# DavidSevic/gpu-nbody-simulation

Hardware: AMD Instinct MI355X
Metric: body-steps/sec (higher is better)
Workload: dtype f32

## Files before the change

gpu-nbody-simulation_amd/csrc/bh_engine.hip:

```cpp
#include "../../include/bhgpu.h"

#include <hip/hip_runtime.h>

#include <algorithm>
#include <chrono>
#include <cmath>
#include <cstdio>
#include <cstdlib>
#include <cstring>
#include <string>
#include <type_traits>
#include <vector>

#include "bh_tree.hpp"
#include "bh_walk_exact.hpp"
#include "bh_walk_f64.hpp"
#include "bh_diag.hpp"
#include "bh_direct.hpp"
#include "bh_field.hpp"
#include "bh_init.hpp"
#include "bh_let.hpp"
#include "bh_migrate.hpp"
#include "bh_split.hpp"
#include "bh_moments.hpp"
#include "bh_radial.hpp"
#include "bh_neighbours.hpp"
#include "bh_pairs.hpp"
#include "bh_groups.hpp"
#include "bh_mst.hpp"
#include "bh_binaries.hpp"
#include "bh_walk_fast.h"
#include "bh_run_state.hpp"
#include "bh_queries_state.hpp"

using namespace bh;

#ifdef BHGPU_EXPERIMENTS
#include "../../scripts/experiments/bh_engine_hooks.hpp"
#else
struct ExpHooks {
    hipError_t create(int64_t) { return hipSuccess; }
    void walk_args(WalkFastArgs &) const {}
    void destroy(int64_t) {}
};
#endif

static thread_local std::string g_create_error;

struct bh_ctx : RunState {
    bh_config cfg{};
    int Dm = 0;
    enum class Mode { Exact, F64, Mixed, F32 };
    Mode mode = Mode::Exact;
    bool tree64() const { return mode == Mode::Exact || mode == Mode::F64; }
    bool state64() const { return mode != Mode::F32; }
    bool compat = true;
    double eps = 0.0, eps2 = 0.0;
    float eps2f = 0.f;
    bool exact_thresholds = false;
    int device = 0;
    hipStream_t stream = nullptr;
    bool own_stream = false;
    int64_t n = 0;
    int64_t internal_cap = 0, node_cap = 0;
    int64_t bfs_max = 12288;
    int exact_bpw = 0;
    int walk_split = 0;
    bool walk_asm = true;
    int sort_bucket = 1;
    uint64_t *splitters = nullptr;
    uint16_t *sort_dig = nullptr;
    int sort_direct = 1;
    int64_t sort_direct_max = kSortDirectMax;
    uint64_t *keys_scatter = nullptr;
    uint64_t *direct_list = nullptr, *direct_range_keys = nullptr;
    uint32_t *direct_count = nullptr;
    uint32_t direct_cap = 0, direct_subcap = 0;
    int direct_nsub = 1;
    int direct_slot = 0;
    struct SortRecord {
        bool valid = false, offered = false;
        int64_t n = 0;
        int nb = 0, nsub = 0;
        uint32_t len = 0, cap = 0, subcap = 0;
        const uint32_t *count = nullptr;
    } sort_rec;
    int build_items = 0;
    bool hilbert = false;
    bool chain_collapse = true;
    double *bslots = nullptr;

    void *pos = nullptr, *vel = nullptr, *mass = nullptr, *force = nullptr;
    void *pos2 = nullptr, *vel2 = nullptr, *mass2 = nullptr, *force2 = nullptr;
    uint32_t *orig = nullptr, *orig2 = nullptr;
    int reorder_every = 16;
    float2 *spos = nullptr;
    float4 *sstate = nullptr;
    float *smass = nullptr;
    uint64_t *keys[2] = {nullptr, nullptr};
    uint32_t *vals[2] = {nullptr, nullptr};
    uint64_t *keys_sorted = nullptr;
    uint32_t *perm = nullptr;
    uint32_t *radix_counts = nullptr, *bsum_sort = nullptr, *bsum_u32 = nullptr, *cnt = nullptr;
    uint64_t *coarse = nullptr;
    uint32_t *cell_first = nullptr;
    d3 *terms = nullptr, *bsum_d3 = nullptr;
    double *partial = nullptr, *box = nullptr;
    NodeD *gd = nullptr;
    LinkD *ld = nullptr;
    QuadF *qf = nullptr;
    NodeAux *aux = nullptr;
    int32_t *self_node = nullptr, *cell_depth = nullptr;
    uint32_t *com_pending = nullptr;
    TreeCounters *ctr = nullptr;

    int rank = 0, world = 1;
    bool let_mode = false, external_box = false;
    int64_t let_cap = 0, quads_local = 0;
    int64_t forest_base = 0;
    uint64_t *needmask = nullptr;
    uint32_t *let_tsum = nullptr, *let_outidx = nullptr;
    QuadF *let_send = nullptr;
    double *lbounds = nullptr, *all_bounds = nullptr;
    float2 *acc_part = nullptr;
    LetCounters *let_ctr = nullptr;
    int64_t *gid = nullptr;
    uint32_t *group_cost = nullptr;
    const void **walk_consts = nullptr;
    uint32_t *body_counts = nullptr;
    double *phi = nullptr;
    uint32_t *phi_counts = nullptr;
    double *diag_part = nullptr, *diag_out = nullptr;
    TsRecord *ts_part = nullptr, *ts_out = nullptr;
    MapState map;
    RadState rad;
    FieldState field;
    NbState nb;
    PairState pair;
    FofState fof;
    MstState mst;
    BinState bin;
    double *slots_save = nullptr;
    TreeCounters *ctr_save = nullptr;
    uint32_t *perm_save = nullptr;
    uint32_t *slot_of = nullptr;
    int64_t *direct_targets = nullptr;
    double2 *direct_out = nullptr;
    void *check_force = nullptr;
    uint32_t *check_counts = nullptr, *check_cost = nullptr;
    bool sort_pack = true;
    unsigned long long *orb_hist = nullptr;
    double *mig_send = nullptr, *mig_recv = nullptr;
    ExpHooks exp;

    std::vector<hipEvent_t> ev;
    hipEvent_t ev_step[2] = {nullptr, nullptr}, ev_build[2] = {nullptr, nullptr};
    hipEvent_t ev_grp[3] = {nullptr, nullptr, nullptr};
    hipEvent_t ev_let[3] = {nullptr, nullptr, nullptr};
    bool let_timed = false;
    int64_t steps_done = 0;
    int32_t last_nsteps = 0;
    int timed_pairs = 0;
    bool step_timed = false;

    std::vector<void *> allocs;
    uint64_t device_bytes = 0;
    std::string err;
};

using Mode = bh_ctx::Mode;
// ... 12 lines not shown
        if (e_ != hipSuccess)                                                                   \
            return fail((c), BH_ERR_DEVICE,                                                     \
                        std::string(#call) + ": " + hipGetErrorString(e_));                     \
    } while (0)

template <typename T>
int dev_alloc(bh_ctx *c, T **out, size_t count)
{
    void *p = nullptr;
    const size_t bytes = std::max<size_t>(count, 1) * sizeof(T);
    hipError_t e = hipMalloc(&p, bytes);
    if (e != hipSuccess)
        return fail(c, BH_ERR_DEVICE, std::string("hipMalloc(") + std::to_string(bytes) + "): " + hipGetErrorString(e));
    c->allocs.push_back(p);
    c->device_bytes += bytes;
    *out = static_cast<T *>(p);
    return BH_OK;
}

inline void dev_free(bh_ctx *c, void *p)
{
    if (!p) return;
    auto it = std::find(c->allocs.begin(), c->allocs.end(), p);
    if (it != c->allocs.end()) { c->allocs.erase(it); (void)hipFree(p); }
}

inline unsigned blocks_for(int64_t n, int per_block) { return (unsigned)((n + per_block - 1) / per_block); }

template <typename F>
void dispatch(F &&f) { f(); }
template <typename F, typename... B>
void dispatch(F &&f, bool b, B... rest)
{
    if (b) dispatch([&](auto... t) { f(std::true_type{}, t...); }, rest...);
    else dispatch([&](auto... t) { f(std::false_type{}, t...); }, rest...);
}

template <typename F>
void with_state(const bh_ctx *c, F &&f)
{
    if (c->state64()) f(double2{}); else f(float2{});
}

inline size_t force_bytes(const bh_ctx *c, int64_t n)
{
    return (size_t)std::max<int64_t>(n, 1) * 2 * (c->tree64() ? sizeof(double) : sizeof(float));
}

inline int64_t cell_span(const bh_ctx *c)
{
    return std::max<int64_t>(1, std::min<int64_t>(c->internal_cap, std::max<int64_t>(c->n - 1, 0) * (int64_t)std::max(1, c->Dm)));
}

void owned_range(const bh_ctx *c, int64_t *lo, int64_t *hi)
{
    if (c->let_mode) { *lo = 0; *hi = c->n; return; }
    const int64_t per = (c->n + c->world - 1) / c->world;
    const int64_t chunk = (per + kBlock - 1) / kBlock * kBlock;
    *lo = std::min<int64_t>(c->n, chunk * c->rank);
    *hi = std::min<int64_t>(c->n, chunk * (c->rank + 1));
}

constexpr int64_t kComClimbMaxBodies = 32768;
constexpr int64_t kSmallBuildBodies = 327680;
constexpr int64_t kMediumBuildBodies = 786432;
constexpr int kSmallItems = 2;

template <typename Real2, typename Real>
__global__ __launch_bounds__(kBlock) void reorder_state_kernel(uint32_t *__restrict__ perm, const Real2 *__restrict__ pos,
                                                                const Real2 *__restrict__ vel, const Real *__restrict__ mass,
                                                                const float2 *__restrict__ acc, const uint32_t *__restrict__ orig,
                                                                Real2 *__restrict__ pos2, Real2 *__restrict__ vel2,
                                                                Real *__restrict__ mass2, float2 *__restrict__ acc2,
                                                                uint32_t *__restrict__ orig2, int64_t n)
{
    const int64_t s = (int64_t)blockIdx.x * kBlock + threadIdx.x;
    if (s >= n) return;
    const uint32_t b = perm[s];
    pos2[s] = pos[b]; vel2[s] = vel[b]; mass2[s] = mass[b]; acc2[s] = acc[b];
    orig2[s] = orig ? orig[b] : b;
    perm[s] = (uint32_t)s;
}

static void launch_nodes_fast(bh_ctx *c, bool full_aux, hipStream_t st)
{
    dispatch([&](auto compat, auto full, auto chains) {
        constexpr bool kCollapse = decltype(chains)::value && !decltype(full)::value;
        hipLaunchKernelGGL((nodes_fast_kernel<decltype(compat)::value, decltype(full)::value, kCollapse>),
                           dim3(blocks_for(cell_span(c), kBlock)),
                           dim3(kBlock), 0, st, c->keys_sorted, c->coarse, c->cnt, c->cell_first, c->spos, c->smass, c->box,
                           c->terms, c->n, c->Dm, c->cfg.theta, c->internal_cap, c->qf, c->aux, c->ctr);
    }, c->compat, full_aux, c->chain_collapse && !(c->let_mode && c->world > 1));
}

void clean_slots(bh_ctx *c) { if (c->carry.slots_dirty) hipLaunchKernelGGL(bounds_slots_reset, dim3(1), dim3(kWave), 0, c->stream, c->bslots); }

template <int SI>
int enqueue_lsd_passes(hipStream_t st, uint64_t *const keys[2], uint32_t *const vals[2], uint32_t *counts, uint32_t *rows, int64_t n,
                       int bits, bool packed)
{
    constexpr int SB = kSortBits;
    const unsigned nbl = blocks_for(n, kBlock * SI);
    const int passes = (bits + SB - 1) / SB;
    int cur = 0;
    for (int p = 0; p < passes; ++p) {
        const int shift = p * SB;
        auto scatter = [&](auto kern) {
            hipLaunchKernelGGL(kern, dim3(nbl), dim3(kBlock), 0, st, keys[cur], packed ? nullptr : vals[cur], keys[cur ^ 1],
                               vals[cur ^ 1], counts, rows, n, shift, (int)nbl, nullptr, nullptr, nullptr, 0u, 0u, 1);
        };
        hipLaunchKernelGGL((radix_hist<SI, SB>), dim3(nbl), dim3(kBlock), 0, st, keys[cur], counts, n, shift, (int)nbl);
        hipLaunchKernelGGL(radix_rowscan, dim3(1 << SB), dim3(kBlock), 0, st, counts, rows, (int)nbl);
        if (!packed) scatter(radix_scatter_w<SI, SB>);
        else if (p + 1 == passes) scatter(radix_scatter_w<SI, SB, 2>);
        else scatter(radix_scatter_w<SI, SB, 1>);
        cur ^= 1;
    }
    return cur;
}

template <bool TREE64, bool STATE64 = TREE64, int ITEMS = kItems>
int enqueue_build_t(bh_ctx *c, bool may_reorder, bool time_groups)
{
    constexpr int TILE = kBlock * ITEMS;
    static_assert(!TREE64 || STATE64, "an fp64 tree is built from fp64 state");
    using Real2 = typename std::conditional<STATE64, double2, float2>::type;
    using Real = typename std::conditional<STATE64, double, float>::type;
    const int64_t n = c->n;
    const int Dm = c->Dm;
    hipStream_t st = c->stream;
    const Real2 *pos = static_cast<const Real2 *>(c->pos);
    const Real *mass = static_cast<const Real *>(c->mass);

    const bool from_walk = c->carry.slots_valid;
    double *slots = c->external_box ? nullptr : c->bslots;
    if (slots) {
        if (!from_walk) {
            const unsigned nbb = std::max(1u, std::min(1024u, blocks_for(n, kBlock)));
            clean_slots(c);
            hipLaunchKernelGGL((bounds_partial<Real2>), dim3(nbb), dim3(kBlock), 0, st, pos, n, slots);
        }
    }
    BuildDone done{n, slots != nullptr, false, false, false, false};

    if (n > 0) {
        const bool pack = Dm >= 1 && 2 * Dm <= kPackShift && n <= ((int64_t)1 << (64 - kPackShift))
                          && c->sort_pack;
        const bool single = pack && n >= 2 && n <= 4 * kBsThreads && c->sort_bucket == 1;
        const bool bucket = !single && pack && n >= 2 && n <= kBucketMaxNBig && (c->sort_bucket == 2 || (c->sort_bucket == 1 && c->carry.samples_n == n));
        const int nb = (n <= kBucketMaxN) ? kBuckets : kBucketsBig;
        const int ns = (nb == kBuckets) ? ((n > (int64_t)1 << 18) ? 2 * kBuckets : kBuckets)
                                        : ((n > (int64_t)3 << 20) ? kMaxSplitSamples : kBucketsBig);
        static_assert(kBucketMaxN == (int64_t)1 << 20 && kBucketMaxNBig == (int64_t)1 << 22, "BASELINE configs 3 and 4 fit");
        done.sort_bucket = bucket || single; done.sort_packed = pack;
        const bool direct = bucket && !TREE64 && c->sort_direct != 0 && c->carry.samples_n == n;
        SortDirect sd;
        BucketDirect bd;
        if (direct) {
            const uint32_t len = (uint32_t)((n + nb - 1) / nb);
            sd.count = c->direct_count + c->direct_slot * kDirectCounterWords;
            sd.count_next = c->direct_count + (c->direct_slot ^ 1) * kDirectCounterWords;
            sd.list = c->direct_list; sd.range_keys = c->direct_range_keys; sd.cap = c->direct_cap; sd.subcap = c->direct_subcap;
            sd.len = len; sd.nsub = c->direct_nsub;
            bd.count = sd.count; bd.list = sd.list; bd.range_keys = sd.range_keys; bd.keys = c->keys[0]; bd.scratch = c->keys_scatter;
            bd.n = n; bd.cap = sd.cap; bd.subcap = sd.subcap; bd.len = len; bd.nb = nb; bd.nsub = sd.nsub;
            c->direct_slot ^= 1;
        }
        {
            const unsigned nkb = blocks_for(n, kBlock);
            auto keys_launch = [&](auto fs, auto pk, auto hil) {
                constexpr bool H = decltype(hil)::value, P = decltype(pk)::value, F = decltype(fs)::value;
                const bool smp = P && bucket;
// ... 401 lines not shown
    kQuietCounters = 1,
    kQuietOutputs = 2,
    kQuietCostPerm = 4,
};

void swap_walk_outputs(bh_ctx *c) { std::swap(c->force, c->check_force); std::swap(c->body_counts, c->check_counts); std::swap(c->group_cost, c->check_cost); }
template <typename Body>
int quietly(bh_ctx *c, unsigned opts, Body body)
{
    constexpr size_t off = offsetof(TreeCounters, visits), ctr_bytes = sizeof(TreeCounters) - off, slot_doubles = (size_t)4 * kBoundSlots;
    if ((opts & kQuietCounters) && !c->ctr_save) { if (int rc = dev_alloc(c, &c->ctr_save, 1)) return rc; }
    if (!c->slots_save) { if (int rc = dev_alloc(c, &c->slots_save, slot_doubles)) return rc; }
    RunState saved = *c;
    if ((opts & kQuietCostPerm) && c->last.group_cost_valid && c->is.tree_valid && !c->last.cost_perm && c->n > 0) {
        if (!c->perm_save) { if (int rc = dev_alloc(c, &c->perm_save, (size_t)std::max<int64_t>(c->cfg.capacity, 1))) return rc; }
        BH_HIP(c, hipMemcpyAsync(c->perm_save, c->perm, (size_t)c->n * sizeof(uint32_t), hipMemcpyDeviceToDevice, c->stream));
        saved.costs_indexed_through(c->perm_save);
    }
    if (opts & kQuietCounters) BH_HIP(c, hipMemcpyAsync((char *)c->ctr_save + off, (char *)c->ctr + off, ctr_bytes, hipMemcpyDeviceToDevice, c->stream));
    BH_HIP(c, hipMemcpyAsync(c->slots_save, c->bslots, slot_doubles * sizeof(double), hipMemcpyDeviceToDevice, c->stream));
    if (opts & kQuietOutputs) swap_walk_outputs(c);
    const int rc = body();
    if (opts & kQuietOutputs) swap_walk_outputs(c);
    c->quiet_end(saved);
    BH_HIP(c, hipMemcpyAsync(c->bslots, c->slots_save, slot_doubles * sizeof(double), hipMemcpyDeviceToDevice, c->stream));
    if (opts & kQuietCounters) BH_HIP(c, hipMemcpyAsync((char *)c->ctr + off, (char *)c->ctr_save + off, ctr_bytes, hipMemcpyDeviceToDevice, c->stream));
    return rc;
}

}

#include "bh_queries_host.hpp"


extern "C" {

int bh_abi_version(void) { return BHGPU_ABI_VERSION; }

#ifndef BHGPU_BUILD_INFO
#define BHGPU_BUILD_INFO "digest=unknown flags=unknown"
#endif
const char *bh_build_info(void) { return BHGPU_BUILD_INFO; }

const char *bh_last_error(const bh_ctx *ctx) { return ctx ? ctx->err.c_str() : g_create_error.c_str(); }

int bh_create(const bh_config *cfg, bh_ctx **out)
{
    if (!cfg || !out) return fail(nullptr, BH_ERR_ARG, "bh_create: null argument");
    *out = nullptr;
    if (cfg->capacity < 0 || cfg->capacity > 0x7fffffffLL - 8)
        return fail(nullptr, BH_ERR_ARG, "bh_create: capacity out of range");
    if (cfg->max_depth < 1 || cfg->max_depth > 32)
        return fail(nullptr, BH_ERR_ARG, "bh_create: max_depth must be 1..32");
    if (!(cfg->theta > 0.0)) return fail(nullptr, BH_ERR_ARG, "bh_create: theta must be > 0");
    if (cfg->precision != BH_PRECISION_F64_EXACT && cfg->precision != BH_PRECISION_F32 &&
        cfg->precision != BH_PRECISION_MIXED && cfg->precision != BH_PRECISION_F64)
        return fail(nullptr, BH_ERR_ARG, "bh_create: unknown precision");
    int ndev = 0;
    if (hipGetDeviceCount(&ndev) != hipSuccess || ndev <= 0)
        return fail(nullptr, BH_ERR_NO_DEVICE, "bh_create: no HIP device (libbhgpu has no CPU fallback)");
    if (cfg->device < 0 || cfg->device >= ndev)
        return fail(nullptr, BH_ERR_ARG, "bh_create: device ordinal out of range");

    bh_ctx *c = new bh_ctx();
    c->cfg = *cfg;
    c->Dm = cfg->max_depth - 1;
    c->mode = cfg->precision == BH_PRECISION_F64_EXACT ? Mode::Exact
            : cfg->precision == BH_PRECISION_F64       ? Mode::F64
            : cfg->precision == BH_PRECISION_MIXED     ? Mode::Mixed : Mode::F32;
    c->compat = cfg->reference_compat != 0;
    c->device = cfg->device;
    if (const char *e = std::getenv("BH_WALK_SPLIT")) c->walk_split = std::atoi(e);
    if (const char *e = std::getenv("BH_EXACT_BPW")) { const int b = std::atoi(e); c->exact_bpw = (b >= 1 && b <= kWave && (b & (b - 1)) == 0) ? b : 0; }
    if (const char *e = std::getenv("BH_WALK_ASM")) c->walk_asm = std::atoi(e) != 0;
    if (const char *e = std::getenv("BH_EXACT_BFS_MAX")) c->bfs_max = std::max(0, std::atoi(e));
    c->exact_thresholds = c->mode == Mode::Exact && c->walk_asm && !(cfg->flags & BH_FLAG_WALK_PORTABLE);
    if (const char *e = std::getenv("BH_SORT_PACK")) c->sort_pack = std::atoi(e) != 0;
    if (const char *e = std::getenv("BH_SORT_BUCKET")) c->sort_bucket = std::atoi(e);
    if (const char *e = std::getenv("BH_SORT_DIRECT")) { const int d = std::atoi(e); c->sort_direct = (d >= 0 && d <= 2) ? d : 1; }
    if (const char *e = std::getenv("BH_SORT_DIRECT_MAX")) c->sort_direct_max = std::max<long long>(0, std::atoll(e));
    if (c->tree64()) c->sort_direct = 0;
    if (const char *e = std::getenv("BH_BUILD_ITEMS")) c->build_items = std::atoi(e);
    if (const char *e = std::getenv("BH_REORDER_EVERY")) c->reorder_every = std::max(0, std::atoi(e));
    c->hilbert = !c->tree64();
    if (const char *e = std::getenv("BH_HILBERT")) c->hilbert = !c->tree64() && std::atoi(e) != 0;
    if (const char *e = std::getenv("BH_CHAIN_COLLAPSE")) c->chain_collapse = std::atoi(e) != 0;
    if (const char *e = std::getenv("BH_RADIAL_BLOCKS")) { const int b = std::atoi(e); if (b >= 1 && b <= 65536) c->rad.blocks = b; }
    auto bail = [&](int rc) { g_create_error = c->err; bh_destroy(c); return rc; };

    if (hipSetDevice(c->device) != hipSuccess) { c->err = "hipSetDevice failed"; return bail(BH_ERR_DEVICE); }
    if (hipStreamCreateWithFlags(&c->stream, hipStreamNonBlocking) != hipSuccess) {
        c->err = "hipStreamCreate failed"; return bail(BH_ERR_DEVICE);
    }
    c->own_stream = true;

    const int64_t cap = std::max<int64_t>(cfg->capacity, 1);
    c->node_cap = cfg->node_capacity > 0 ? cfg->node_capacity : 8 * cap + 1024;
    if (c->Dm < 15) {
        int64_t full = 0, wdt = 1;
        for (int l = 0; l <= c->Dm; ++l) { full += wdt; wdt *= 4; }
        c->node_cap = std::min(c->node_cap, std::max<int64_t>(full, 1));
    }
    c->internal_cap = (c->node_cap - 1) / 4;

    const size_t rs = c->state64() ? sizeof(double) : sizeof(float);
    int rc = 0;
    auto A = [&](auto **pp, size_t count) { if (!rc) rc = dev_alloc(c, pp, count); };
    { char *t; A(&t, cap * 2 * rs); c->pos = t; }
    { char *t; A(&t, cap * 2 * rs); c->vel = t; }
    { char *t; A(&t, cap * rs); c->mass = t; }
    { char *t; A(&t, force_bytes(c, cap)); c->force = t; }
    if (!c->tree64()) {
        { char *t; A(&t, cap * 2 * rs); c->pos2 = t; }
        { char *t; A(&t, cap * 2 * rs); c->vel2 = t; }
        { char *t; A(&t, cap * rs); c->mass2 = t; }
        { char *t; A(&t, cap * 2 * sizeof(float)); c->force2 = t; }
        A(&c->orig, cap); A(&c->orig2, cap);
    }
    A(&c->keys[0], cap); A(&c->keys[1], cap); A(&c->vals[0], cap); A(&c->vals[1], cap);
    A(&c->cnt, cap + 1);
    { const size_t nbl = std::max<size_t>(blocks_for(cap, kSortTile), blocks_for(std::min<int64_t>(cap, 1 << 22), kBlock * kSmallItems));
      const size_t big = (cap > kBucketMaxN) ? (size_t)kBucketsBig * blocks_for(std::min<int64_t>(cap, kBucketMaxNBig), kBlock * kSmallItems) : 0;
      A(&c->radix_counts, std::max<size_t>((size_t)(1 << kSortBits) * nbl, big));
      A(&c->bsum_sort, 2 * kBucketStartOffset);
      A(&c->splitters, kBucketsBig);
      A(&c->sort_dig, (size_t)std::min<int64_t>(cap, kBucketMaxNBig) + 16);
      if (c->sort_direct) {
          const int64_t most = std::min<int64_t>(cap, kBucketMaxNBig);
          c->direct_cap = (uint32_t)std::min<int64_t>(most, c->sort_direct == 2 ? most : c->sort_direct_max);
          c->direct_nsub = c->sort_direct == 2 ? 1 : kDirectSubs;
          c->direct_subcap = c->direct_cap;
          if (c->sort_direct != 2) { c->direct_subcap = 16; while ((int64_t)c->direct_subcap * (kDirectSubs / 4) < c->direct_cap) c->direct_subcap *= 2; }
          A(&c->keys_scatter, (size_t)most);
          A(&c->direct_list, std::max<size_t>((size_t)c->direct_nsub * c->direct_subcap, 1));
          A(&c->direct_range_keys, kBucketsBig);
          A(&c->direct_count, 2 * kDirectCounterWords);
      }
    }
    const size_t scan_tiles = std::max<size_t>(blocks_for(cap + 1, kTile), blocks_for(std::min<int64_t>(cap, 1 << 22) + 1, kBlock * kSmallItems)) + 8;
    A(&c->bsum_u32, scan_tiles);
    A(&c->partial, 4 * (std::max<size_t>(1024, blocks_for(cap, kWave)) + 2));
    A(&c->box, 8); A(&c->bslots, 4 * kBoundSlots);
    A(&c->ctr, 1);
    if (c->tree64()) {
        { NodeD *g0 = nullptr; LinkD *l0 = nullptr; A(&g0, c->node_cap + 4); A(&l0, c->node_cap + 4);
          if (!rc) { c->gd = g0 + 3; c->ld = l0 + 3; } }
        A(&c->self_node, c->internal_cap + 1); A(&c->com_pending, c->internal_cap + 1); A(&c->cell_depth, c->internal_cap + 1);
        A(&c->cell_first, c->internal_cap + 1);
    } else {
        A(&c->qf, c->internal_cap + 1); A(&c->aux, 4 * (c->internal_cap + 1));
        A(&c->cell_first, c->internal_cap + 1);
        A(&c->gid, cap); A(&c->group_cost, cap / kWave + 2); A(&c->walk_consts, 4);
        A(&c->coarse, cap / 256 + 2);
        A(&c->spos, cap); A(&c->sstate, cap + 64 * kBlock + 1024); A(&c->smass, cap);
        A(&c->terms, cap + 1); A(&c->bsum_d3, scan_tiles);
    }
    if (rc) return bail(rc);
    if (hipMemset(c->ctr, 0, sizeof(TreeCounters)) != hipSuccess) { c->err = "hipMemset failed"; return bail(BH_ERR_DEVICE); }
    if (c->direct_count && hipMemset(c->direct_count, 0, 2 * kDirectCounterWords * sizeof(uint32_t)) != hipSuccess) { c->err = "hipMemset failed"; return bail(BH_ERR_DEVICE); }
    if (!c->tree64()) {
        const void *wc[4] = {c->aux, c->spos, c->smass, nullptr};
        if (hipMemcpy(c->walk_consts, wc, sizeof(wc), hipMemcpyHostToDevice) != hipSuccess) { c->err = "hipMemcpy failed"; return bail(BH_ERR_DEVICE); }
    }
    if (!c->tree64() && c->exp.create(cap) != hipSuccess) { c->err = "experiment hooks: allocation failed"; return bail(BH_ERR_DEVICE); }
    auto create = [](auto &evs) { for (auto &e : evs) if (hipEventCreate(&e) != hipSuccess) return false; return true; };
    if (!create(c->ev_step) || !create(c->ev_build) || !create(c->ev_grp) || !create(c->ev_let)) {
        c->err = "hipEventCreate failed"; return bail(BH_ERR_DEVICE);
    }
    *out = c;
    return BH_OK;
}

void bh_destroy(bh_ctx *c)
// ... 1217 lines not shown
```

gpu-nbody-simulation_amd/csrc/bh_tree.hpp:

```cpp
#pragma once

#include <type_traits>

#include "bh_prims.hpp"
#include "bh_sort.hpp"
#include "bh_nodes.hpp"
#include "bh_bounds.hpp"

namespace bh {

constexpr int kCoarse = 256;

__device__ __forceinline__ int shared_levels(uint64_t a, uint64_t b, int Dm)
{
    const uint64_t x = a ^ b;
    if (x == 0) return Dm;
    return (__clzll((long long)x) - (64 - 2 * Dm)) >> 1;
}

template <typename Real2>
__global__ __launch_bounds__(kBlock) void bounds_partial(const Real2 *__restrict__ pos, int64_t n, double *slots)
{
    double xlo = INFINITY, xhi = -INFINITY, ylo = INFINITY, yhi = -INFINITY;
    for (int64_t i = (int64_t)blockIdx.x * kBlock + threadIdx.x; i < n; i += (int64_t)gridDim.x * kBlock) {
// ... 684 lines not shown
        kprev[c] = (sub4[c] && bc4[c] > 0) ? keys[bc4[c] - 1] : 0ull;
    }
    double m1[4];
    double2 p1[4];
#pragma unroll
    for (int c = 0; c < 4; ++c) {
        m1[c] = one4[c] ? mass[bi1[c]] : 0.0;
        p1[c] = one4[c] ? pos[bi1[c]] : double2{0.0, 0.0};
    }
#pragma unroll
    for (int c = 0; c < 4; ++c) {
        const double cx0 = (c & 1) ? mx : x0, cx1 = (c & 1) ? x1 : mx;
        const double cy0 = (c & 2) ? my : y0, cy1 = (c & 2) ? y1 : my;
        const double ex = cx1 - cx0, ey = cy1 - cy0;
        const double size = (ex > ey) ? ex : ey;
        const int64_t bc = bc4[c], nc = nc4[c];
        const int32_t node = quad + c;
        double m = 0.0, cx = 0.0, cy = 0.0;
        int32_t child = -1, occ = -1;
        if (nc == 0) {
        } else if (d + 1 == Dm) {
            for (int64_t j = bc; j < bc + nc; ++j) {
                const uint32_t bi = perm[j];
                const double bm = mass[bi], bx = pos[bi].x, by = pos[bi].y;
                cx = (m * cx + bm * bx) / (m + bm);
                cy = (m * cy + bm * by) / (m + bm);
                m += bm;
            }
            occ = (nc == 1) ? (-(int32_t)perm[bc] - 2) : -1;
        } else if (nc == 1) {
            m = m1[c]; cx = p1[c].x; cy = p1[c].y;
            occ = (int32_t)bi1[c];
        } else {
            const int Lpc = (bc == 0) ? -1 : shared_levels(kprev[c], kcur[c], Dm);
            const uint32_t rc = offc[c] + (uint32_t)((d + 1) - (Lpc + 1));
            child = 1 + 4 * (int32_t)rc;
            self_node[rc] = node;
            ++n_sub;
        }
        double *sn = s_nd + threadIdx.x * 16 + 4 * c;
        sn[0] = cx; sn[1] = cy; sn[2] = m; sn[3] = size_slot(size);
        s_ln[threadIdx.x * 8 + 2 * c] = child; s_ln[threadIdx.x * 8 + 2 * c + 1] = occ;
    }
    pending[r] = n_sub;
    }
    __syncthreads();
    {
        const int64_t left = (int64_t)total - r_block;
        const int cells = (left < kBlock) ? (int)left : kBlock;
        double2 *dn = reinterpret_cast<double2 *>(gd + 1 + 4 * r_block);
        const double2 *sn = reinterpret_cast<const double2 *>(s_nd);
        for (int k = threadIdx.x; k < cells * 8; k += kBlock) dn[k] = sn[k];
        int2 *dl = reinterpret_cast<int2 *>(ld + 1 + 4 * r_block);
        const int2 *sl = reinterpret_cast<const int2 *>(s_ln);
        for (int k = threadIdx.x; k < cells * 4; k += kBlock) dl[k] = sl[k];
    }
}

constexpr int kMaxBucket = 1024;
constexpr int kKeyHalo = 768;
constexpr int kKeyWin = kBlock + 1 + kKeyHalo;

template <bool COMPAT, bool FULL_AUX = false, bool COLLAPSE = false>
__global__ __launch_bounds__(kBlock, 5) void nodes_fast_kernel(
    const uint64_t *__restrict__ keys, const uint64_t *__restrict__ coarse,
    const uint32_t *__restrict__ off, const uint32_t *__restrict__ cell_first,
    const float2 *__restrict__ spos,
    const float *__restrict__ smass, const double *__restrict__ box, const d3 *__restrict__ psum,
    int64_t n64, int Dm, double theta, int64_t internal_cap, QuadF *__restrict__ qf,
    NodeAux *__restrict__ aux, TreeCounters *ctr)
{
    static_assert(!(FULL_AUX && COLLAPSE), "the exported tree keeps every link");
    constexpr int kStageBytes = kBlock * (FULL_AUX ? 28 : 20) * 4, kWinBytes = kKeyWin * 8;
    __shared__ __attribute__((aligned(16))) unsigned char lds_raw[kStageBytes > kWinBytes ? kStageBytes : kWinBytes];
    uint64_t *wkeys = reinterpret_cast<uint64_t *>(lds_raw);
    __shared__ int32_t s_wlo;
    __shared__ double s_thr0;
    int32_t *stage_q = reinterpret_cast<int32_t *>(lds_raw);
    int32_t *stage_a = stage_q + kBlock * 20;
    const int32_t n = (int32_t)n64;
    const uint32_t total = ctr->n_internal;
    float *qw = reinterpret_cast<float *>(qf);
    int32_t *qi = reinterpret_cast<int32_t *>(qf);
    auto put = [&](int32_t quad, int slot, float cx, float cy, float m, float thr, int32_t child) {
        const int64_t o = (int64_t)quad * 20;
        qw[o + 2 * slot] = cx; qw[o + 2 * slot + 1] = cy; qw[o + 8 + slot] = m; qw[o + 12 + slot] = thr;
        qi[o + 16 + slot] = child;
    };
    auto put_lds = [&](int slot, float cx, float cy, float m, float thr, int32_t child) {
        int32_t *o = stage_q + threadIdx.x * 20;
        o[2 * slot] = __float_as_int(cx); o[2 * slot + 1] = __float_as_int(cy);
        o[8 + slot] = __float_as_int(m); o[12 + slot] = __float_as_int(thr); o[16 + slot] = child;
    };

    if (total == 0) {
        if (blockIdx.x == 0 && threadIdx.x == 0) {
            for (int k = 0; k < 4; ++k) { put(0, k, 0.f, 0.f, 0.f, -1.f, -1); aux[k] = NodeAux{0, 0}; }
            if (n >= 1) {
                const d3 t = psum[n];
                const bool one = (n == 1);
                const float cx = one ? spos[0].x : (float)(t.b / t.a), cy = one ? spos[0].y : (float)(t.c / t.a);
                const float m = (t.a > 1e-15) ? (one ? smass[0] : (float)t.a) : 0.f;
                const bool bucket = (n > 1) && (n <= kMaxBucket) && !COMPAT;
                put(0, 0, cx, cy, m, bucket ? INFINITY : 0.f, bucket ? -2 : -1);
                aux[0] = NodeAux{0, (int32_t)n};
            }
        }
        return;
    }
    if ((int64_t)total > internal_cap) {
        if (blockIdx.x == 0 && threadIdx.x == 0) ctr->overflow = 1;
        return;
    }
    const uint32_t r_block = blockIdx.x * kBlock;
    if (r_block >= total) return;

    const uint32_t r = r_block + threadIdx.x;
    const int32_t i_pre = (r < total) ? (int32_t)cell_first[r] : 0;
    const uint32_t off_pre = (r < total) ? off[i_pre] : 0u;

    if (threadIdx.x == 0) {
        s_wlo = i_pre - 1;
        const double ex0 = box[1] - box[0], ey0 = box[3] - box[2];
        const double q0 = ((ex0 > ey0) ? ex0 : ey0) / theta;
        s_thr0 = q0 * q0;
    }
    __syncthreads();
    const int32_t wlo = s_wlo;
    for (int k = threadIdx.x; k < kKeyWin; k += kBlock) {
        const int32_t j = wlo + k;
        wkeys[k] = (j >= 0 && j < n) ? keys[j] : 0ull;
    }
    __syncthreads();
    auto K = [&](int32_t j) -> uint64_t {
        const int32_t k = j - wlo;
        const bool in = (uint32_t)k < (uint32_t)kKeyWin;
        uint64_t v = wkeys[in ? k : 0];
        if (__ballot(!in) != 0ull) {
            asm volatile("" : "+v"(v));
            if (!in) v = keys[j];
        }
        return v;
    };

    auto search = [&](auto nt_tag, auto keyfn, int32_t lo0, int32_t hi0, int sh, const uint64_t *target, int32_t *res) {
        constexpr int NT = decltype(nt_tag)::value;
        int32_t lo[NT], hi[NT];
#pragma unroll
        for (int c = 0; c < NT; ++c) { lo[c] = lo0; hi[c] = hi0; }
        if (hi0 - lo0 > 4 * kCoarse) {
            int32_t cl[NT], ch[NT];
            bool more = true;
#pragma unroll
            for (int c = 0; c < NT; ++c) { cl[c] = (lo0 + kCoarse - 1) / kCoarse; ch[c] = (hi0 - 1) / kCoarse + 1; }
            while (more) {
                uint64_t k1[NT], k2[NT], k3[NT];
                int32_t p1[NT], p2[NT], p3[NT];
#pragma unroll
                for (int c = 0; c < NT; ++c) {
                    const int32_t len = ch[c] - cl[c];
                    p1[c] = cl[c] + len / 4; p2[c] = cl[c] + len / 2; p3[c] = cl[c] + (int32_t)((3 * (int64_t)len) / 4);
                    const bool on = len > 0;
                    k1[c] = on ? coarse[p1[c]] : 0ull; k2[c] = on ? coarse[p2[c]] : 0ull; k3[c] = on ? coarse[p3[c]] : 0ull;
                }
                more = false;
#pragma unroll
                for (int c = 0; c < NT; ++c) {
                    if (ch[c] - cl[c] > 0) {
                        if ((k1[c] >> sh) >= target[c]) ch[c] = p1[c];
                        else if ((k2[c] >> sh) >= target[c]) { cl[c] = p1[c] + 1; ch[c] = p2[c]; }
                        else if ((k3[c] >> sh) >= target[c]) { cl[c] = p2[c] + 1; ch[c] = p3[c]; }
                        else cl[c] = p3[c] + 1;
                    }
                    more = more || (ch[c] - cl[c] > 0);
                }
            }
#pragma unroll
            for (int c = 0; c < NT; ++c) {
                const int32_t up = (cl[c] * kCoarse < hi0) ? cl[c] * kCoarse : hi0;
                const int32_t dn = ((cl[c] - 1) * kCoarse > lo0) ? (cl[c] - 1) * kCoarse : lo0;
                lo[c] = dn; hi[c] = up;
            }
        }
        bool more = true;
        while (more) {
            uint64_t k2[NT];
            int32_t p2[NT];
#pragma unroll
            for (int c = 0; c < NT; ++c) {
                p2[c] = (int32_t)(((uint32_t)lo[c] + (uint32_t)hi[c]) >> 1);
                k2[c] = (hi[c] > lo[c]) ? keyfn(p2[c]) : 0ull;
            }
            more = false;
#pragma unroll
            for (int c = 0; c < NT; ++c) {
                if (hi[c] > lo[c]) {
                    if ((k2[c] >> sh) >= target[c]) hi[c] = p2[c]; else lo[c] = p2[c] + 1;
                }
                more = more || (hi[c] > lo[c]);
            }
        }
#pragma unroll
        for (int c = 0; c < NT; ++c) res[c] = lo[c];
    };
    auto lower_bound = [&](int32_t lo, int32_t hi, int sh, uint64_t target) -> int32_t {
        int32_t r;
        search(std::integral_constant<int, 1>{}, K, lo, hi, sh, &target, &r);
        return r;
    };

    float res_cx[4], res_cy[4], res_m[4], res_thr[4];
    int32_t res_child[4], res_bc[4], res_nc[4];
    if (r < total) {
    const int32_t i = i_pre;
    const uint64_t key = K(i);
    const int Lp = (i == 0) ? -1 : shared_levels(K(i - 1), key, Dm);
    const int d = Lp + 1 + (int)(r - off_pre);

    const double thr0 = s_thr0;

    const int sh = 2 * (Dm - d);
    const uint64_t pfx = (d == 0) ? 0ull : (key >> sh);
    int32_t e;
    int32_t bnd[5];
    bool have_bnd = false;
    const int shc = sh - 2;
    if (d == 0) e = n;
    else {
        const uint64_t cell_hi = (pfx + 1) << sh;
        uint64_t nk[8];
#pragma unroll
        for (int j = 0; j < 8; ++j) nk[j] = 0ull;
        const int32_t k1 = i + 1 - wlo;
        if (__ballot(!(k1 >= 0 && k1 + 8 <= kKeyWin && i + 8 < n)) == 0ull) {
#pragma unroll
            for (int j = 0; j < 8; ++j) nk[j] = wkeys[k1 + j];
        } else {
#pragma unroll
            for (int j = 0; j < 8; ++j) nk[j] = (i + 1 + j < n) ? K(i + 1 + j) : ~0ull;
        }
        int inside = 0;
#pragma unroll
        for (int j = 0; j < 8; ++j) inside += (nk[j] < cell_hi) ? 1 : 0;
        if (inside < 8) {
            e = i + 1 + inside;
            int below1 = 0, below2 = 0, below3 = 0;
            {
                const uint32_t dg = (uint32_t)(key >> shc) & 3u;
                below1 += dg < 1u; below2 += dg < 2u; below3 += dg < 3u;
            }
#pragma unroll
            for (int j = 0; j < 8; ++j) {
                const uint32_t dg = (j < inside) ? (uint32_t)(nk[j] >> shc) & 3u : 3u;
                below1 += dg < 1u; below2 += dg < 2u; below3 += dg < 3u;
            }
            bnd[1] = i + below1; bnd[2] = i + below2; bnd[3] = i + below3;
            have_bnd = true;
        }
    }
    if (d != 0 && !have_bnd) {
        int32_t a = i + 8, step = 8, b;
        for (;;) {
            b = (step > n - a) ? n : a + step;
            if (b >= n) { b = n; break; }
            if (step > 2 * kCoarse) break;
            if ((K(b) >> sh) != pfx) break;
            a = b; step <<= 1;
        }
        if (step > 2 * kCoarse && b < n && (K(b) >> sh) == pfx) { a = b; b = n; }
        e = lower_bound(a + 1, b, sh, pfx + 1);
    }
    const int32_t quad = (int32_t)r + 1;

    if (d == 0) {
        for (int k = 1; k < 4; ++k) { put(0, k, 0.f, 0.f, 0.f, -1.f, -1); aux[k] = NodeAux{0, 0}; }
        const d3 t = psum[n];
        int dz0 = 0;
        if (COLLAPSE) { const int s0 = shared_levels(key, K(n - 1), Dm); dz0 = (s0 < Dm - 1) ? s0 : Dm - 1; }
        if (t.a > 1e-15) put(0, 0, (float)(t.b / t.a), (float)(t.c / t.a), (float)t.a, (float)ldexp(thr0, -2 * dz0), quad + dz0);
        else put(0, 0, 0.f, 0.f, 0.f, -1.f, -1);
        aux[0] = NodeAux{0, n};
    }
    const float thr_child = (float)ldexp(thr0, -2 * (d + 1));

    bnd[0] = i; bnd[4] = e;
    auto KF = [&](int32_t j) -> uint64_t { return wkeys[j - wlo]; };
    const bool cells_in_window = __ballot(!(i - 1 >= wlo && e - wlo <= kKeyWin)) == 0ull;
    if (!have_bnd) {
        const uint64_t tg[3] = {(pfx << 2) | 1ull, (pfx << 2) | 2ull, (pfx << 2) | 3ull};
        if (cells_in_window) {
            int32_t lo3[3] = {i, i, i}, hi3[3] = {e, e, e};
            const uint64_t t3[3] = {tg[0] << shc, tg[1] << shc, tg[2] << shc};
            while ((hi3[0] > lo3[0]) | (hi3[1] > lo3[1]) | (hi3[2] > lo3[2])) {
#pragma unroll
                for (int c = 0; c < 3; ++c) {
                    const int32_t pm = (int32_t)(((uint32_t)lo3[c] + (uint32_t)hi3[c]) >> 1);
                    const uint64_t km = wkeys[pm - wlo];
                    const bool open = hi3[c] > lo3[c], ge = km >= t3[c];
                    hi3[c] = (open && ge) ? pm : hi3[c];
                    lo3[c] = (open && !ge) ? pm + 1 : lo3[c];
                }
            }
            bnd[1] = lo3[0]; bnd[2] = lo3[1]; bnd[3] = lo3[2];
        }
        else search(std::integral_constant<int, 3>{}, K, i, e, shc, tg, &bnd[1]);
    }
    d3 ps[5];
    uint32_t offc[4];
    uint64_t kprev[4], kcur[4], klast[4];
    float2 p1[4];
    float m1[4];
#pragma unroll
    for (int c = 0; c < 5; ++c) {
        bool left = c > 0 && bnd[c] - bnd[c - 1] > 1, right = c < 4 && bnd[c + 1] - bnd[c] > 1;
        ps[c] = (left || right) ? psum[bnd[c]] : d3{1.0, 1.0, 1.0};
    }
#pragma unroll
    for (int c = 0; c < 4; ++c) {
        const int32_t bc = bnd[c];
        const int32_t ncc = bnd[c + 1] - bc;
        const bool sub = ncc > 1 && d + 1 < Dm;
        offc[c] = sub ? off[bc] : 0u;
        if (cells_in_window) {
            kcur[c] = sub ? KF(bc) : 0ull;
            kprev[c] = (sub && bc > 0) ? KF(bc - 1) : 0ull;
            klast[c] = (COLLAPSE && sub) ? KF(bnd[c + 1] - 1) : 0ull;
        } else {
            kcur[c] = sub ? K(bc) : 0ull;
            kprev[c] = (sub && bc > 0) ? K(bc - 1) : 0ull;
            klast[c] = (COLLAPSE && sub) ? K(bnd[c + 1] - 1) : 0ull;
        }
        p1[c] = (ncc == 1) ? spos[bc] : float2{0.f, 0.f};
        m1[c] = (ncc == 1) ? smass[bc] : 0.f;
    }
#pragma unroll
    for (int c = 0; c < 4; ++c) {
        const int32_t bc = bnd[c], bn = bnd[c + 1];
        const int32_t nc = bn - bc;
        float cx = 0.f, cy = 0.f, m = 0.f, thr = 0.f;
        int32_t child = -1;
        if (nc == 1) {
            cx = p1[c].x; cy = p1[c].y; m = m1[c];
        } else if (nc > 1) {
            const d3 lo_s = ps[c], hi_s = ps[c + 1];
            const double mm = hi_s.a - lo_s.a;
            double inv = __builtin_amdgcn_rcp(mm);
            inv = fma(fma(-mm, inv, 1.0), inv, inv);
            inv = fma(fma(-mm, inv, 1.0), inv, inv);
            m = (float)mm; cx = (float)((hi_s.b - lo_s.b) * inv); cy = (float)((hi_s.c - lo_s.c) * inv);
            if (d + 1 == Dm) {
                if (!COMPAT && nc <= kMaxBucket) { thr = INFINITY; child = -(4 * quad + c) - 2; }
            } else {
                const int Lpc = (bc == 0) ? -1 : shared_levels(kprev[c], kcur[c], Dm);
                child = (int32_t)(offc[c] + (uint32_t)((d + 1) - (Lpc + 1))) + 1;
                thr = thr_child;
                if (COLLAPSE) {
                    const int sl = shared_levels(kcur[c], klast[c], Dm);
                    const int dz = (sl < Dm - 1) ? sl : Dm - 1;
                    child += dz - (d + 1);
                    thr = (float)ldexp(thr0, -2 * dz);
                }
            }
        }
        if (!(m > 1e-15f)) { cx = 0.f; cy = 0.f; m = 0.f; thr = 0.f; child = -1; }
        res_cx[c] = cx; res_cy[c] = cy; res_m[c] = m; res_thr[c] = thr; res_child[c] = child;
        res_bc[c] = bc; res_nc[c] = nc;
    }
    }

    __syncthreads();
    if (r < total) {
#pragma unroll
        for (int c = 0; c < 4; ++c) {
            put_lds(c, res_cx[c], res_cy[c], res_m[c], res_thr[c], res_child[c]);
            if (FULL_AUX) {
                stage_a[threadIdx.x * 8 + 2 * c] = res_bc[c];
                stage_a[threadIdx.x * 8 + 2 * c + 1] = res_nc[c];
            } else if (res_child[c] <= -2) {
                aux[4 * ((int64_t)r + 1) + c] = NodeAux{res_bc[c], res_nc[c]};
            }
        }
    }
    __syncthreads();
    const uint32_t cells = (total - r_block < (uint32_t)kBlock) ? total - r_block : (uint32_t)kBlock;
    {
        typedef int32_t v4 __attribute__((ext_vector_type(4)));
        v4 *dq = reinterpret_cast<v4 *>(qi + ((int64_t)r_block + 1) * 20);
        const v4 *sq = reinterpret_cast<const v4 *>(stage_q);
        for (uint32_t k = threadIdx.x; k < cells * 5; k += kBlock) dq[k] = sq[k];
        if (FULL_AUX) {
            v4 *da = reinterpret_cast<v4 *>(aux + 4 * ((int64_t)r_block + 1));
            const v4 *sa = reinterpret_cast<const v4 *>(stage_a);
            for (uint32_t k = threadIdx.x; k < cells * 2; k += kBlock) da[k] = sa[k];
        }
    }
}

__global__ __launch_bounds__(kBlock) void com_up_kernel(NodeD *__restrict__ gd, const LinkD *__restrict__ ld,
                                                         const int32_t *__restrict__ self_node,
                                                         uint32_t *__restrict__ pending,
                                                         const TreeCounters *__restrict__ ctr, int64_t internal_cap)
{
    const int64_t r0 = (int64_t)blockIdx.x * kBlock + threadIdx.x;
    const uint32_t total = ctr->n_internal;
    if (r0 >= (int64_t)total || (int64_t)total > internal_cap) return;
    if (pending[r0] != 0) return;
    uint32_t r = (uint32_t)r0;
    for (;;) {
        const int32_t node = self_node[r];
        const int32_t quad = 1 + 4 * (int32_t)r;
        double tot = 0.0, sx = 0.0, sy = 0.0;
#pragma unroll
        for (int c = 0; c < 4; ++c) {
            const double cm = __hip_atomic_load(&gd[quad + c].m, __ATOMIC_RELAXED, __HIP_MEMORY_SCOPE_AGENT);
            const double cx = __hip_atomic_load(&gd[quad + c].cx, __ATOMIC_RELAXED, __HIP_MEMORY_SCOPE_AGENT);
            const double cy = __hip_atomic_load(&gd[quad + c].cy, __ATOMIC_RELAXED, __HIP_MEMORY_SCOPE_AGENT);
            tot += cm;
            sx += cm * cx;
            sy += cm * cy;
        }
        if (tot > 0.0) { sx /= tot; sy /= tot; }
        __hip_atomic_store(&gd[node].cx, sx, __ATOMIC_RELAXED, __HIP_MEMORY_SCOPE_AGENT);
        __hip_atomic_store(&gd[node].cy, sy, __ATOMIC_RELAXED, __HIP_MEMORY_SCOPE_AGENT);
        __hip_atomic_store(&gd[node].m, tot, __ATOMIC_RELAXED, __HIP_MEMORY_SCOPE_AGENT);
        if (r == 0) break;
        const uint32_t parent = (uint32_t)(node - 1) >> 2;
        const uint32_t left = __hip_atomic_fetch_sub(&pending[parent], 1u, __ATOMIC_ACQ_REL, __HIP_MEMORY_SCOPE_AGENT);
        if (left != 1u) break;
        r = parent;
    }
}

__global__ __launch_bounds__(kBlock) void com_level_kernel(NodeD *__restrict__ gd, const int32_t *__restrict__ self_node,
                                                            const int32_t *__restrict__ cell_depth,
                                                            const TreeCounters *__restrict__ ctr, int64_t internal_cap,
                                                            int depth)
{
    const int64_t r = (int64_t)blockIdx.x * kBlock + threadIdx.x;
    const uint32_t total = ctr->n_internal;
    if (r >= (int64_t)total || (int64_t)total > internal_cap) return;
    if (cell_depth[r] != depth) return;
    const int32_t node = self_node[r];
    const int32_t quad = 1 + 4 * (int32_t)r;
    double tot = 0.0, sx = 0.0, sy = 0.0;
#pragma unroll
    for (int c = 0; c < 4; ++c) {
        const NodeD ch = gd[quad + c];
        tot += ch.m;
        sx += ch.m * ch.cx;
        sy += ch.m * ch.cy;
    }
    if (tot > 0.0) { sx /= tot; sy /= tot; }
    gd[node].cx = sx; gd[node].cy = sy; gd[node].m = tot;
}

}
```

Before: 2.505 billion.

## Make tree node kernel persistent grid-stride with prefetched key window

The node-construction kernel now launches a grid capped at a multiple of the CU count and loops over tiles grid-stride style. While the current tile is processed, it prefetches the next tile's cell_first, offsets and key window into registers, then stores them to LDS after the tile finishes. The root-node initialisation moves out of the per-cell path. This aims to cut launch/tail overhead and hide global load latency, but it adds extra barriers and register pressure per tile.

```diff
diff --git a/gpu-nbody-simulation_amd/csrc/bh_engine.hip b/gpu-nbody-simulation_amd/csrc/bh_engine.hip
--- a/gpu-nbody-simulation_amd/csrc/bh_engine.hip
+++ b/gpu-nbody-simulation_amd/csrc/bh_engine.hip
@@ -86,6 +86,8 @@
         const uint32_t *count = nullptr;
     } sort_rec;
     int build_items = 0;
+    int cu_count = 0;
+    int nodes_grid = 0;
     bool hilbert = false;
     bool chain_collapse = true;
     double *bslots = nullptr;
@@ -264,12 +266,16 @@
     perm[s] = (uint32_t)s;
 }
 
+constexpr int kNodesResident = 5, kNodesGridRounds = 8;
 static void launch_nodes_fast(bh_ctx *c, bool full_aux, hipStream_t st)
 {
+    const unsigned tiles = blocks_for(cell_span(c), kBlock);
+    const unsigned want = c->nodes_grid > 0 ? (unsigned)c->nodes_grid : (unsigned)(kNodesGridRounds * kNodesResident * std::max(1, c->cu_count));
+    const unsigned grid = std::max(1u, std::min(tiles, want));
     dispatch([&](auto compat, auto full, auto chains) {
         constexpr bool kCollapse = decltype(chains)::value && !decltype(full)::value;
         hipLaunchKernelGGL((nodes_fast_kernel<decltype(compat)::value, decltype(full)::value, kCollapse>),
-                           dim3(blocks_for(cell_span(c), kBlock)),
+                           dim3(grid),
                            dim3(kBlock), 0, st, c->keys_sorted, c->coarse, c->cnt, c->cell_first, c->spos, c->smass, c->box,
                            c->terms, c->n, c->Dm, c->cfg.theta, c->internal_cap, c->qf, c->aux, c->ctr);
     }, c->compat, full_aux, c->chain_collapse && !(c->let_mode && c->world > 1));
@@ -837,6 +843,7 @@
     if (c->tree64()) c->sort_direct = 0;
     if (const char *e = std::getenv("BH_BUILD_ITEMS")) c->build_items = std::atoi(e);
     if (const char *e = std::getenv("BH_REORDER_EVERY")) c->reorder_every = std::max(0, std::atoi(e));
+    if (const char *e = std::getenv("BH_NODES_GRID")) c->nodes_grid = std::max(0, std::atoi(e));
     c->hilbert = !c->tree64();
     if (const char *e = std::getenv("BH_HILBERT")) c->hilbert = !c->tree64() && std::atoi(e) != 0;
     if (const char *e = std::getenv("BH_CHAIN_COLLAPSE")) c->chain_collapse = std::atoi(e) != 0;
@@ -844,6 +851,9 @@
     auto bail = [&](int rc) { g_create_error = c->err; bh_destroy(c); return rc; };
 
     if (hipSetDevice(c->device) != hipSuccess) { c->err = "hipSetDevice failed"; return bail(BH_ERR_DEVICE); }
+    if (hipDeviceGetAttribute(&c->cu_count, hipDeviceAttributeMultiprocessorCount, c->device) != hipSuccess || c->cu_count < 1) {
+        c->err = "hipDeviceGetAttribute(multiprocessor count) failed"; return bail(BH_ERR_DEVICE);
+    }
     if (hipStreamCreateWithFlags(&c->stream, hipStreamNonBlocking) != hipSuccess) {
         c->err = "hipStreamCreate failed"; return bail(BH_ERR_DEVICE);
     }
diff --git a/gpu-nbody-simulation_amd/csrc/bh_tree.hpp b/gpu-nbody-simulation_amd/csrc/bh_tree.hpp
--- a/gpu-nbody-simulation_amd/csrc/bh_tree.hpp
+++ b/gpu-nbody-simulation_amd/csrc/bh_tree.hpp
@@ -790,13 +790,14 @@
     const uint32_t total = ctr->n_internal;
     float *qw = reinterpret_cast<float *>(qf);
     int32_t *qi = reinterpret_cast<int32_t *>(qf);
+    uint32_t tid = threadIdx.x;
     auto put = [&](int32_t quad, int slot, float cx, float cy, float m, float thr, int32_t child) {
         const int64_t o = (int64_t)quad * 20;
         qw[o + 2 * slot] = cx; qw[o + 2 * slot + 1] = cy; qw[o + 8 + slot] = m; qw[o + 12 + slot] = thr;
         qi[o + 16 + slot] = child;
     };
     auto put_lds = [&](int slot, float cx, float cy, float m, float thr, int32_t child) {
-        int32_t *o = stage_q + threadIdx.x * 20;
+        int32_t *o = stage_q + tid * 20;
         o[2 * slot] = __float_as_int(cx); o[2 * slot + 1] = __float_as_int(cy);
         o[8 + slot] = __float_as_int(m); o[12 + slot] = __float_as_int(thr); o[16 + slot] = child;
     };
@@ -820,26 +821,53 @@
         if (blockIdx.x == 0 && threadIdx.x == 0) ctr->overflow = 1;
         return;
     }
-    const uint32_t r_block = blockIdx.x * kBlock;
-    if (r_block >= total) return;
-
-    const uint32_t r = r_block + threadIdx.x;
-    const int32_t i_pre = (r < total) ? (int32_t)cell_first[r] : 0;
-    const uint32_t off_pre = (r < total) ? off[i_pre] : 0u;
-
+    uint32_t rb = blockIdx.x;
+    if ((uint64_t)rb * kBlock >= total) return;
+    constexpr int kWinRows = (kKeyWin + kBlock - 1) / kBlock;
+
+    uint32_t r = rb * kBlock + threadIdx.x;
+    int32_t i_pre = (r < total) ? (int32_t)cell_first[r] : 0;
     if (threadIdx.x == 0) {
-        s_wlo = i_pre - 1;
         const double ex0 = box[1] - box[0], ey0 = box[3] - box[2];
         const double q0 = ((ex0 > ey0) ? ex0 : ey0) / theta;
         s_thr0 = q0 * q0;
     }
+    uint32_t off_pre = (r < total) ? off[i_pre] : 0u;
+    if (threadIdx.x == 0) s_wlo = i_pre - 1;
     __syncthreads();
-    const int32_t wlo = s_wlo;
-    for (int k = threadIdx.x; k < kKeyWin; k += kBlock) {
-        const int32_t j = wlo + k;
-        wkeys[k] = (j >= 0 && j < n) ? keys[j] : 0ull;
-    }
+    int32_t wlo = __builtin_amdgcn_readfirstlane(s_wlo);
+    uint64_t wnext[kWinRows];
+    auto load_window = [&](int32_t w0) {
+#pragma unroll
+        for (int k = 0; k < kWinRows; ++k) {
+            const int32_t kk = (int)tid + k * kBlock, j = w0 + kk;
+            const int32_t jc = (j < 0) ? 0 : (j < n ? j : n - 1);
+            wnext[k] = 0ull;
+            if ((k + 1) * kBlock <= kKeyWin || kk < kKeyWin) wnext[k] = keys[jc];
+        }
+    };
+    auto store_window = [&](int32_t w0) {
+#pragma unroll
+        for (int k = 0; k < kWinRows; ++k) {
+            const int32_t kk = (int)tid + k * kBlock, j = w0 + kk;
+            if ((k + 1) * kBlock <= kKeyWin || kk < kKeyWin) wkeys[kk] = (j >= 0 && j < n) ? wnext[k] : 0ull;
+        }
+    };
+    load_window(wlo);
+    if (r == 0)
+        for (int k = 1; k < 4; ++k) { put(0, k, 0.f, 0.f, 0.f, -1.f, -1); aux[k] = NodeAux{0, 0}; }
+    store_window(wlo);
     __syncthreads();
+
+    for (;;) {
+    asm volatile("" : "+v"(tid));
+    const uint32_t r_block = rb * kBlock;
+    const uint32_t rb_next = rb + gridDim.x;
+    const bool has_next = (uint64_t)rb_next * kBlock < total;
+    const uint32_t r_next = rb_next * kBlock + tid;
+    const bool cell_next = has_next && r_next < total;
+    const int32_t i_next = cell_next ? (int32_t)cell_first[r_next] : 0;
+    uint32_t off_next = 0u;
     auto K = [&](int32_t j) -> uint64_t {
         const int32_t k = j - wlo;
         const bool in = (uint32_t)k < (uint32_t)kKeyWin;
@@ -917,8 +945,8 @@
         return r;
     };
 
-    float res_cx[4], res_cy[4], res_m[4], res_thr[4];
-    int32_t res_child[4], res_bc[4], res_nc[4];
+    float res_cx[4] = {}, res_cy[4] = {}, res_m[4] = {}, res_thr[4] = {};
+    int32_t res_child[4] = {}, res_bc[4] = {}, res_nc[4] = {};
     if (r < total) {
     const int32_t i = i_pre;
     const uint64_t key = K(i);
@@ -981,11 +1009,14 @@
     const int32_t quad = (int32_t)r + 1;
 
     if (d == 0) {
-        for (int k = 1; k < 4; ++k) { put(0, k, 0.f, 0.f, 0.f, -1.f, -1); aux[k] = NodeAux{0, 0}; }
         const d3 t = psum[n];
         int dz0 = 0;
         if (COLLAPSE) { const int s0 = shared_levels(key, K(n - 1), Dm); dz0 = (s0 < Dm - 1) ? s0 : Dm - 1; }
-        if (t.a > 1e-15) put(0, 0, (float)(t.b / t.a), (float)(t.c / t.a), (float)t.a, (float)ldexp(thr0, -2 * dz0), quad + dz0);
+        int tiny_hi = 0x3cd203af, tiny_lo = (int)0x9ee75616u;
+        asm volatile("" : "+v"(tiny_hi), "+v"(tiny_lo));
+        const double tiny = __hiloint2double(tiny_hi, tiny_lo);
+        static_assert(1e-15 == 0x1.203af9ee75616p-50, "the two words above");
+        if (t.a > tiny) put(0, 0, (float)(t.b / t.a), (float)(t.c / t.a), (float)t.a, (float)ldexp(thr0, -2 * dz0), quad + dz0);
         else put(0, 0, 0.f, 0.f, 0.f, -1.f, -1);
         aux[0] = NodeAux{0, n};
     }
@@ -1018,6 +1049,7 @@
     uint64_t kprev[4], kcur[4], klast[4];
     float2 p1[4];
     float m1[4];
+    if (cell_next) off_next = off[i_next];
 #pragma unroll
     for (int c = 0; c < 5; ++c) {
         bool left = c > 0 && bnd[c] - bnd[c - 1] > 1, right = c < 4 && bnd[c + 1] - bnd[c] > 1;
@@ -1076,14 +1108,16 @@
     }
     }
 
+    if (has_next && tid == 0) s_wlo = i_next - 1;
     __syncthreads();
+    const int32_t wlo_next = __builtin_amdgcn_readfirstlane(s_wlo);
     if (r < total) {
 #pragma unroll
         for (int c = 0; c < 4; ++c) {
             put_lds(c, res_cx[c], res_cy[c], res_m[c], res_thr[c], res_child[c]);
             if (FULL_AUX) {
-                stage_a[threadIdx.x * 8 + 2 * c] = res_bc[c];
-                stage_a[threadIdx.x * 8 + 2 * c + 1] = res_nc[c];
+                stage_a[tid * 8 + 2 * c] = res_bc[c];
+                stage_a[tid * 8 + 2 * c + 1] = res_nc[c];
             } else if (res_child[c] <= -2) {
                 aux[4 * ((int64_t)r + 1) + c] = NodeAux{res_bc[c], res_nc[c]};
             }
@@ -1095,12 +1129,19 @@
         typedef int32_t v4 __attribute__((ext_vector_type(4)));
         v4 *dq = reinterpret_cast<v4 *>(qi + ((int64_t)r_block + 1) * 20);
         const v4 *sq = reinterpret_cast<const v4 *>(stage_q);
-        for (uint32_t k = threadIdx.x; k < cells * 5; k += kBlock) dq[k] = sq[k];
+        for (uint32_t k = tid; k < cells * 5; k += kBlock) dq[k] = sq[k];
         if (FULL_AUX) {
             v4 *da = reinterpret_cast<v4 *>(aux + 4 * ((int64_t)r_block + 1));
             const v4 *sa = reinterpret_cast<const v4 *>(stage_a);
-            for (uint32_t k = threadIdx.x; k < cells * 2; k += kBlock) da[k] = sa[k];
-        }
+            for (uint32_t k = tid; k < cells * 2; k += kBlock) da[k] = sa[k];
+        }
+    }
+    if (!has_next) break;
+    load_window(wlo_next);
+    rb = rb_next; r = r_next; i_pre = i_next; off_pre = off_next; wlo = wlo_next;
+    __syncthreads();
+    store_window(wlo);
+    __syncthreads();
     }
 }
 
```

New measurement: 2.485 billion. No clear change (-0.8%).
